# nihaomiao/CVPR23_LFDM

Measured on AMD Instinct MI355X. Metric: 40-frame 128x128 videos/sec (DDIM-100), higher is better.
Workload: dtype f32; 1 GPU; MUG 128x128, 40-frame DDIM-100 sample, batch=1 per GPU (BASELINE.json configs[1]); global_batch=1, frames=40, latent=32, image=128, sampler=DDIM-100 eta=1, cond_scale=1, parallelism=replicas x1 (videos sharded, no collective)

## Files before the change

cvpr23_lfdm_amd/csrc/lfdm_device.h:

```cpp
#pragma once
#include <stddef.h>
#include <stdint.h>
#include <type_traits>

#if defined(LFDM_EMU_BUILD)
#include "hip_emu.h"
typedef emu_f32x16 f32x16;
typedef emu_f32x4 f32x4;
#define LFDM_LAUNCH(kern, grid, block, smem, stream, ...) \
  emu::launch(grid, block, smem, [=]() { kern(__VA_ARGS__); })
static inline f32x16 mfma_32x32x2(float a, float b, f32x16 c) { return emu_mfma_32x32x2(a, b, c); }
static inline f32x4 mfma_16x16x4(float a, float b, f32x4 c) { return emu_mfma_16x16x4(a, b, c); }
static inline f32x4 mfma_4x4x1(float a, float b, f32x4 c) { return emu_mfma_4x4x1(a, b, c); }
struct lfdm_bf16x8 { uint16_t h[8]; };
static inline uint16_t lfdm_f32_to_bf16(float f) {
  uint32_t u;
  memcpy(&u, &f, 4);
  if ((u & 0x7fffffffu) > 0x7f800000u) return (uint16_t)((u >> 16) | 0x40u);
  u += 0x7fffu + ((u >> 16) & 1u);
  return (uint16_t)(u >> 16);
}
static inline float lfdm_bf16_to_f32(uint16_t h) {
  const uint32_t u = (uint32_t)h << 16;
  float f;
// ... 99 lines not shown
}
__device__ __forceinline__ float4 lfdm_buf_load_f4(lfdm_buf b, uint32_t off) {
  const lfdm_i32x4 v = __builtin_amdgcn_raw_buffer_load_b128(b, (int)off, 0, 0);
  float4 f;
  f.x = __int_as_float(v.x);
  f.y = __int_as_float(v.y);
  f.z = __int_as_float(v.z);
  f.w = __int_as_float(v.w);
  return f;
}
typedef int lfdm_i32x2 __attribute__((ext_vector_type(2)));
__device__ __forceinline__ float2 lfdm_buf_load_f2(lfdm_buf b, uint32_t off) {
  const lfdm_i32x2 v = __builtin_amdgcn_raw_buffer_load_b64(b, (int)off, 0, 0);
  return make_float2(__int_as_float(v.x), __int_as_float(v.y));
}
#endif
#define LFDM_BUF_OOB 0xFFFFFFF0u

#if defined(LFDM_EMU_BUILD)
static inline void lfdm_buf_store_f4_sc1(lfdm_buf b, uint32_t off, float4 v) {
  if ((uint64_t)off + 16u <= (uint64_t)b.bytes) memcpy(const_cast<char*>(b.base) + off, &v, 16);
}
static inline float4 lfdm_buf_load_f4_sc1(lfdm_buf b, uint32_t off) { return lfdm_buf_load_f4(b, off); }
#else
__device__ __forceinline__ void lfdm_buf_store_f4_sc1(lfdm_buf b, uint32_t off, float4 v) {
  lfdm_i32x4 d;
  d.x = __float_as_int(v.x); d.y = __float_as_int(v.y); d.z = __float_as_int(v.z); d.w = __float_as_int(v.w);
  __builtin_amdgcn_raw_buffer_store_b128(d, b, (int)off, 0, 16);
}
__device__ __forceinline__ float4 lfdm_buf_load_f4_sc1(lfdm_buf b, uint32_t off) {
  const lfdm_i32x4 v = __builtin_amdgcn_raw_buffer_load_b128(b, (int)off, 0, 16);
  float4 f;
  f.x = __int_as_float(v.x); f.y = __int_as_float(v.y); f.z = __int_as_float(v.z); f.w = __int_as_float(v.w);
  return f;
}
#endif

#if defined(LFDM_EMU_BUILD)
template <int OFF = 0> static inline void lfdm_gload_f4(f32x4& dst, const float* p) { memcpy(&dst, (const char*)p + OFF, 16); }
template <int N> static inline void lfdm_vmwait() {}
template <int N> static inline void lfdm_vmwait(f32x4&) {}
template <int N> static inline void lfdm_vmwait(f32x4&, f32x4&) {}
template <int N> static inline void lfdm_vmwait(f32x4&, f32x4&, f32x4&, f32x4&) {}
static inline void lfdm_tie(f32x4&) {}
static inline int lfdm_uniform(int v) { return v; }
#else
template <int OFF = 0>
__device__ __forceinline__ void lfdm_gload_f4(f32x4& dst, const float* p) {
  asm volatile("global_load_dwordx4 %0, %1, off offset:%2" : "=v"(dst) : "v"(p), "n"(OFF) : "memory");
}
template <int N> __device__ __forceinline__ void lfdm_vmwait() { asm volatile("s_waitcnt vmcnt(%0)" ::"n"(N) : "memory"); }
template <int N> __device__ __forceinline__ void lfdm_vmwait(f32x4& a) { asm volatile("s_waitcnt vmcnt(%1)" : "+v"(a) : "n"(N) : "memory"); }
template <int N> __device__ __forceinline__ void lfdm_vmwait(f32x4& a, f32x4& b) {
  asm volatile("s_waitcnt vmcnt(%2)" : "+v"(a), "+v"(b) : "n"(N) : "memory");
}
template <int N> __device__ __forceinline__ void lfdm_vmwait(f32x4& a, f32x4& b, f32x4& c, f32x4& d) {
  asm volatile("s_waitcnt vmcnt(%4)" : "+v"(a), "+v"(b), "+v"(c), "+v"(d) : "n"(N) : "memory");
// ... 87 lines not shown
```

cvpr23_lfdm_amd/csrc/linattn_fused.hip:

```cpp
#include <stdlib.h>

#include "lfdm_device.h"
#include "../../include/lfdm_hip.h"

namespace {

constexpr int HEADS = 8;
constexpr int DH = 32;
constexpr int OUT_LD = HEADS * DH;
constexpr int C = 64;
constexpr int CH = C / 2;
constexpr int SPLIT_TOK = 32;
constexpr int PART = DH * DH + 2 * DH;
constexpr float LA_SCALE = 0.17677669529663687f;

__device__ __forceinline__ void load_xraw(const float* __restrict__ xrow, int kh, float4 (&raw)[CH / 4]) {
#pragma unroll
  for (int q = 0; q < CH / 4; ++q) raw[q] = *reinterpret_cast<const float4*>(xrow + CH * kh + 4 * q);
}
__device__ __forceinline__ void xhat_stats(const float4 (&raw)[CH / 4], float eps, float& mean, float& rstd) {
  float s1 = 0.f, s2 = 0.f;
#pragma unroll
  for (int q = 0; q < CH / 4; ++q) {
    const float4 v = raw[q];
    s1 += (v.x + v.y) + (v.z + v.w);
    s2 += (v.x * v.x + v.y * v.y) + (v.z * v.z + v.w * v.w);
  }
  s1 += __shfl_xor(s1, 32);
  s2 += __shfl_xor(s2, 32);
  mean = s1 * (1.0f / (float)C);
  float var = s2 * (1.0f / (float)C) - mean * mean;
  if (var < 0.f) var = 0.f;
  rstd = 1.0f / sqrtf(var + eps);
}
__device__ __forceinline__ void xhat_apply(const float4 (&raw)[CH / 4], bool ok, float mean, float rstd, float (&xf)[CH]) {
#pragma unroll
// ... 2 lines not shown
    xf[4 * q] = ok ? (v.x - mean) * rstd : 0.f;
    xf[4 * q + 1] = ok ? (v.y - mean) * rstd : 0.f;
    xf[4 * q + 2] = ok ? (v.z - mean) * rstd : 0.f;
    xf[4 * q + 3] = ok ? (v.w - mean) * rstd : 0.f;
  }
}
__device__ __forceinline__ void load_xhat(const float* __restrict__ xrow, bool ok, int kh, float eps, float (&xf)[CH]) {
  float4 raw[CH / 4];
  float mean, rstd;
  load_xraw(xrow, kh, raw);
  xhat_stats(raw, eps, mean, rstd);
  xhat_apply(raw, ok, mean, rstd, xf);
}

__device__ __forceinline__ void load_wfrag(const float* __restrict__ wp, int which, int head, int lane, float (&wf)[CH]) {
  const float* src = wp + ((int64_t)(which * HEADS + head) * (CH / 4) * 64 + lane) * 4;
#pragma unroll
  for (int q = 0; q < CH / 4; ++q) {
    const float4 v = *reinterpret_cast<const float4*>(src + 256 * q);
    wf[4 * q] = v.x; wf[4 * q + 1] = v.y; wf[4 * q + 2] = v.z; wf[4 * q + 3] = v.w;
  }
}

__global__ __launch_bounds__(64, 3) void linattn_fused_ctx_kernel(const float* __restrict__ x, int ldx,
                                                                  const float* __restrict__ wqkv, int hw, float eps,
                                                                  float* __restrict__ part, int split_tok) {
  const int lane = threadIdx.x & 63, l31 = lane & 31, kh = lane >> 5;
  const int f = blockIdx.x >> 3, h = blockIdx.x & 7;
  const int split = blockIdx.y, nsplit = gridDim.y;
  const int n0 = split * split_tok;
  const int n1 = (n0 + split_tok < hw) ? n0 + split_tok : hw;

  float wk[CH], wv[CH];
  load_wfrag(wqkv, 1, h, lane, wk);
  load_wfrag(wqkv, 2, h, lane, wv);

  float m_run = -3.0e38f, s_run = 0.f;
  f32x16 ctx;
#pragma unroll
  for (int r = 0; r < 16; ++r) ctx[r] = 0.f;
  for (int t0 = n0; t0 < n1; t0 += 32) {
    const int n = t0 + l31;
    float xf[CH];
    load_xhat(x + ((int64_t)f * hw + (n < n1 ? n : n1 - 1)) * ldx, n < n1, kh, eps, xf);
    f32x16 ka, va;
#pragma unroll
    for (int r = 0; r < 16; ++r) ka[r] = va[r] = 0.f;
#pragma unroll
    for (int s = 0; s < CH; ++s) {
      ka = mfma_32x32x2(xf[s], wk[s], ka);
      va = mfma_32x32x2(xf[s], wv[s], va);
// ... 3 lines not shown
    for (int r = 0; r < 16; ++r) {
      const int tok = t0 + (r & 3) + 8 * (r >> 2) + 4 * kh;
      if (tok < n1) m = fmaxf(m, ka[r]);
    }
    m = fmaxf(m, __shfl_xor(m, 32));
    const float m_new = fmaxf(m_run, m);
    const float alpha = expf(m_run - m_new);
    float ssum = 0.f;
    float e[16];
#pragma unroll
    for (int r = 0; r < 16; ++r) {
      const int tok = t0 + (r & 3) + 8 * (r >> 2) + 4 * kh;
      e[r] = tok < n1 ? expf(ka[r] - m_new) : 0.f;
      ssum += e[r];
    }
    ssum += __shfl_xor(ssum, 32);
    s_run = s_run * alpha + ssum;
    m_run = m_new;
#pragma unroll
    for (int r = 0; r < 16; ++r) ctx[r] *= __shfl(alpha, (r & 3) + 8 * (r >> 2) + 4 * kh);
#pragma unroll
    for (int r = 0; r < 16; ++r) ctx = mfma_32x32x2(e[r], va[r], ctx);
  }
  float* dst = part + ((int64_t)blockIdx.x * nsplit + split) * PART;
#pragma unroll
  for (int r = 0; r < 16; ++r) dst[((r & 3) + 8 * (r >> 2) + 4 * kh) * DH + l31] = ctx[r];
  if (kh == 0) {
    dst[DH * DH + l31] = m_run;
    dst[DH * DH + DH + l31] = s_run;
  }
}

__global__ __launch_bounds__(256) void linattn_fused_merge_kernel(const float* __restrict__ part, int nsplit,
                                                                  float* __restrict__ ctx_out) {
  constexpr int MAXS = 64;
  __shared__ float s_w[MAXS][DH];
  const int tid = threadIdx.x;
  const float* base = part + (int64_t)blockIdx.x * nsplit * PART;
  if (nsplit <= 8) {
    constexpr int PS = 8;
    float cv[4][PS], pm[PS], psum[PS];
#pragma unroll
    for (int p = 0; p < PS; ++p) {
      const int pc = p < nsplit ? p : nsplit - 1;
#pragma unroll
      for (int e = 0; e < 4; ++e) cv[e][p] = base[(int64_t)pc * PART + tid + 256 * e];
      pm[p] = base[(int64_t)pc * PART + DH * DH + (tid & (DH - 1))];
      psum[p] = base[(int64_t)pc * PART + DH * DH + DH + (tid & (DH - 1))];
    }
    if (tid < DH) {
      float mm = -3.0e38f;
#pragma unroll
      for (int p = 0; p < PS; ++p)
        if (p < nsplit) mm = fmaxf(mm, pm[p]);
      float den = 0.f, w[PS];
#pragma unroll
      for (int p = 0; p < PS; ++p) {
        w[p] = p < nsplit ? expf(pm[p] - mm) : 0.f;
        den += w[p] * psum[p];
      }
      const float inv = 1.0f / den;
#pragma unroll
      for (int p = 0; p < PS; ++p)
        if (p < nsplit) s_w[p][tid] = w[p] * inv;
    }
    __syncthreads();
#pragma unroll
    for (int e = 0; e < 4; ++e) {
      const int i = tid + 256 * e, d = i >> 5;
      float acc = 0.f;
#pragma unroll
      for (int p = 0; p < PS; ++p)
        if (p < nsplit) acc += s_w[p][d] * cv[e][p];
      ctx_out[(int64_t)blockIdx.x * DH * DH + i] = acc;
    }
    return;
  }
  if (tid < DH) {
    float mm = -3.0e38f;
#pragma unroll 4
    for (int p = 0; p < nsplit; ++p) mm = fmaxf(mm, base[(int64_t)p * PART + DH * DH + tid]);
    float den = 0.f;
#pragma unroll 4
    for (int p = 0; p < nsplit; ++p) {
      const float w = expf(base[(int64_t)p * PART + DH * DH + tid] - mm);
      s_w[p][tid] = w;
      den += w * base[(int64_t)p * PART + DH * DH + DH + tid];
    }
    const float inv = 1.0f / den;
    for (int p = 0; p < nsplit; ++p) s_w[p][tid] *= inv;
  }
  __syncthreads();
  for (int i = tid; i < DH * DH; i += 256) {
    const int d = i >> 5;
    float acc = 0.f;
#pragma unroll 4
    for (int p = 0; p < nsplit; ++p) acc += s_w[p][d] * base[(int64_t)p * PART + i];
    ctx_out[(int64_t)blockIdx.x * DH * DH + i] = acc;
  }
}

__global__ __launch_bounds__(64, 2) void linattn_fused_out_kernel(const float* __restrict__ x, int ldx,
                                                                  const float* __restrict__ wqkv,
                                                                  const float* __restrict__ ctx, int hw, float eps,
                                                                  float* __restrict__ out) {
  const int lane = threadIdx.x & 63, l31 = lane & 31, kh = lane >> 5;
  const int f = blockIdx.y;
  const int n = blockIdx.x * 32 + l31;
  float xf[CH];
  load_xhat(x + ((int64_t)f * hw + (n < hw ? n : 0)) * ldx, n < hw, kh, eps, xf);
  const int hpb = HEADS / gridDim.z;
#pragma unroll 1
  for (int h = blockIdx.z * hpb; h < (blockIdx.z + 1) * hpb; ++h) {
    float wq[CH];
    load_wfrag(wqkv, 0, h, lane, wq);
    f32x16 q;
#pragma unroll
    for (int r = 0; r < 16; ++r) q[r] = 0.f;
#pragma unroll
    for (int s = 0; s < CH; ++s) q = mfma_32x32x2(wq[s], xf[s], q);
    float m = q[0];
#pragma unroll
    for (int r = 1; r < 16; ++r) m = fmaxf(m, q[r]);
    m = fmaxf(m, __shfl_xor(m, 32));
    float sum = 0.f;
#pragma unroll
    for (int r = 0; r < 16; ++r) {
      q[r] = expf(q[r] - m);
      sum += q[r];
    }
    sum += __shfl_xor(sum, 32);
    const float inv = LA_SCALE / sum;
    const float* cb = ctx + ((int64_t)f * HEADS + h) * DH * DH + l31;
    f32x16 o;
#pragma unroll
    for (int r = 0; r < 16; ++r) o[r] = 0.f;
#pragma unroll
    for (int r = 0; r < 16; ++r) o = mfma_32x32x2(q[r] * inv, cb[((r & 3) + 8 * (r >> 2) + 4 * kh) * DH], o);
#pragma unroll
    for (int r = 0; r < 16; ++r) {
      const int tok = blockIdx.x * 32 + (r & 3) + 8 * (r >> 2) + 4 * kh;
      if (tok < hw) out[((int64_t)f * hw + tok) * OUT_LD + h * DH + l31] = o[r];
    }
  }
}


constexpr int LDY = C + 4;
__global__ __launch_bounds__(256, 2) void linattn_fused_out2_kernel(const float* __restrict__ x, int ldx, const float* __restrict__ wqkv,
                                                                    const float* __restrict__ wout, const float* __restrict__ bias_out,
                                                                    const float* __restrict__ ctx, int hw, float eps, float* __restrict__ out,
                                                                    int ldo) {
  __shared__ __attribute__((aligned(16))) float s_y[4 * 32 * LDY];
  const int tid = threadIdx.x;
  const int wave = lfdm_uniform(tid >> 6);
  const int lane = tid & 63, l31 = lane & 31, kh = lane >> 5;
  const int f = blockIdx.y;
  const int n0 = blockIdx.x * 32;
  const int n = n0 + l31;
  float xf[CH];
  load_xhat(x + ((int64_t)f * hw + (n < hw ? n : 0)) * ldx, n < hw, kh, eps, xf);
  f32x16 yT[2];
#pragma unroll
  for (int cb = 0; cb < 2; ++cb)
#pragma unroll
    for (int r = 0; r < 16; ++r) yT[cb][r] = 0.f;
#pragma unroll 1
  for (int h = 2 * wave; h < 2 * wave + 2; ++h) {
    float wq[CH];
    load_wfrag(wqkv, 0, h, lane, wq);
    f32x16 q;
#pragma unroll
    for (int r = 0; r < 16; ++r) q[r] = 0.f;
#pragma unroll
    for (int s = 0; s < CH; ++s) q = mfma_32x32x2(wq[s], xf[s], q);
    float m = q[0];
#pragma unroll
    for (int r = 1; r < 16; ++r) m = fmaxf(m, q[r]);
    m = fmaxf(m, __shfl_xor(m, 32));
    float sum = 0.f;
#pragma unroll
    for (int r = 0; r < 16; ++r) {
      q[r] = expf(q[r] - m);
      sum += q[r];
    }
    sum += __shfl_xor(sum, 32);
    const float inv = LA_SCALE / sum;
    const float* cb_ = ctx + ((int64_t)f * HEADS + h) * DH * DH + l31;
    f32x16 oT;
#pragma unroll
    for (int r = 0; r < 16; ++r) oT[r] = 0.f;
#pragma unroll
    for (int r = 0; r < 16; ++r) oT = mfma_32x32x2(cb_[((r & 3) + 8 * (r >> 2) + 4 * kh) * DH], q[r] * inv, oT);
#pragma unroll
    for (int cb = 0; cb < 2; ++cb) {
      const float* wsrc = wout + ((int64_t)((h * 2 + cb) * 4) * 64 + lane) * 4;
      float4 wo[4];
#pragma unroll
      for (int qd = 0; qd < 4; ++qd) wo[qd] = *reinterpret_cast<const float4*>(wsrc + 256 * qd);
#pragma unroll
      for (int qd = 0; qd < 4; ++qd) {
        yT[cb] = mfma_32x32x2(wo[qd].x, oT[4 * qd + 0], yT[cb]);
        yT[cb] = mfma_32x32x2(wo[qd].y, oT[4 * qd + 1], yT[cb]);
        yT[cb] = mfma_32x32x2(wo[qd].z, oT[4 * qd + 2], yT[cb]);
        yT[cb] = mfma_32x32x2(wo[qd].w, oT[4 * qd + 3], yT[cb]);
      }
    }
  }
  float* ys = s_y + (wave * 32 + l31) * LDY;
#pragma unroll
  for (int cb = 0; cb < 2; ++cb)
#pragma unroll
    for (int g = 0; g < 4; ++g)
      *reinterpret_cast<float4*>(ys + 32 * cb + 8 * g + 4 * kh) = make_float4(yT[cb][4 * g], yT[cb][4 * g + 1], yT[cb][4 * g + 2], yT[cb][4 * g + 3]);
  __syncthreads();
  const int tok = tid >> 3, c8 = (tid & 7) * 8;
  if (n0 + tok < hw) {
    const int64_t row = (int64_t)f * hw + n0 + tok;
#pragma unroll
    for (int j = 0; j < 2; ++j) {
      const int c = c8 + 4 * j;
      float4 v = *reinterpret_cast<const float4*>(x + row * ldx + c);
      const float4 b4 = bias_out ? *reinterpret_cast<const float4*>(bias_out + c) : make_float4(0.f, 0.f, 0.f, 0.f);
      v.x += b4.x; v.y += b4.y; v.z += b4.z; v.w += b4.w;
#pragma unroll
      for (int w4 = 0; w4 < 4; ++w4) {
        const float4 u = *reinterpret_cast<const float4*>(s_y + (w4 * 32 + tok) * LDY + c);
        v.x += u.x; v.y += u.y; v.z += u.z; v.w += u.w;
      }
      *reinterpret_cast<float4*>(out + row * ldo + c) = v;
    }
  }
}

}

extern "C" size_t lfdm_linear_attention_fused_ws_bytes(int n_frames, int hw) {
  const int nsplit = (hw + SPLIT_TOK - 1) / SPLIT_TOK;
  return ((size_t)n_frames * HEADS * nsplit * PART + (size_t)n_frames * HEADS * DH * DH) * sizeof(float);
}

namespace {
void launch_ctx_and_merge(const float* x, int ldx, const float* wqkv, int n_frames, int hw, float ln_eps, void* ws, float** ctx_out,
                          hipStream_t stream) {
  const int tiles = (hw + 31) / 32;
  const int64_t pairs = (int64_t)n_frames * HEADS;
  int want = (int)((pairs <= 1536 ? 3072 : 4 * 3072 + pairs - 1) / pairs);
  if (const char* e = lfdm_knob("LFDM_LINATTN_SPLITS")) want = atoi(e);
  if (want < 1) want = 1;
  if (want > 64) want = 64;
  if (want > tiles) want = tiles;
  const int split_tok = ((tiles + want - 1) / want) * 32;
  const int nsplit = (hw + split_tok - 1) / split_tok;
  float* part = (float*)ws;
  float* ctx = part + (size_t)n_frames * HEADS * ((hw + SPLIT_TOK - 1) / SPLIT_TOK) * PART;
  LFDM_LAUNCH(linattn_fused_ctx_kernel, dim3(n_frames * HEADS, nsplit), dim3(64), 0, stream, x, ldx, wqkv, hw, ln_eps, part, split_tok);
  LFDM_LAUNCH(linattn_fused_merge_kernel, dim3(n_frames * HEADS), dim3(256), 0, stream, (const float*)part, nsplit, ctx);
  *ctx_out = ctx;
}
}

extern "C" int lfdm_linear_attention_fused_cl_f32(const float* x, int ldx, int channels, const float* wqkv, float* out,
                                                  int n_frames, int hw, float ln_eps, void* ws, size_t ws_bytes,
                                                  lfdm_stream_t stream_) {
  hipStream_t stream = (hipStream_t)stream_;
  if (!x || !wqkv || !out || n_frames <= 0 || hw <= 0 || hw > 64 * 64 || channels != C || ldx < C || ldx % 4 != 0 ||
      (((uintptr_t)x | (uintptr_t)wqkv) & 15) || (int64_t)n_frames * HEADS > 0x7fffffff) {
    lfdm_set_error("linear_attention_fused: needs C == 64 and 16-byte aligned rows");
    return LFDM_EINVAL;
  }
  if (!ws || ws_bytes < lfdm_linear_attention_fused_ws_bytes(n_frames, hw)) {
    lfdm_set_error("linear_attention_fused: workspace too small");
    return LFDM_EWORKSPACE;
  }
  float* ctx = nullptr;
  launch_ctx_and_merge(x, ldx, wqkv, n_frames, hw, ln_eps, ws, &ctx, stream);
  const int64_t otiles = (int64_t)((hw + 31) / 32) * n_frames;
  const int hgroups = otiles >= 4096 ? 1 : (otiles >= 2048 ? 2 : 4);
  LFDM_LAUNCH(linattn_fused_out_kernel, dim3((hw + 31) / 32, n_frames, hgroups), dim3(64), 0, stream, x, ldx, wqkv,
              (const float*)ctx, hw, ln_eps, out);
  return lfdm_check_launch("linear_attention_fused");
}

extern "C" int lfdm_linear_attention_fused_out_cl_f32(const float* x, int ldx, int channels, const float* wqkv, const float* wout,
                                                      const float* bias_out, float* out, int ldo, int n_frames, int hw, float ln_eps,
                                                      void* ws, size_t ws_bytes, lfdm_stream_t stream_) {
  hipStream_t stream = (hipStream_t)stream_;
  if (!x || !wqkv || !wout || !out || out == x || n_frames <= 0 || hw <= 0 || hw > 64 * 64 || channels != C || ldx < C || ldx % 4 != 0 || ldo < C ||
      ldo % 4 != 0 || (((uintptr_t)x | (uintptr_t)wqkv | (uintptr_t)wout | (uintptr_t)out | (uintptr_t)bias_out) & 15) ||
      (int64_t)n_frames * HEADS > 0x7fffffff || n_frames > 65535) {
    lfdm_set_error("linear_attention_fused_out: needs C == 64, 16-byte aligned rows, out != x, <= 65535 frames");
    return LFDM_EINVAL;
  }
  if (!ws || ws_bytes < lfdm_linear_attention_fused_ws_bytes(n_frames, hw)) {
    lfdm_set_error("linear_attention_fused_out: workspace too small");
    return LFDM_EWORKSPACE;
  }
  float* ctx = nullptr;
  launch_ctx_and_merge(x, ldx, wqkv, n_frames, hw, ln_eps, ws, &ctx, stream);
  LFDM_LAUNCH(linattn_fused_out2_kernel, dim3((hw + 31) / 32, n_frames), dim3(256), 0, stream, x, ldx, wqkv, wout, bias_out, (const float*)ctx, hw,
              ln_eps, out, ldo);
  return lfdm_check_launch("linear_attention_fused_out");
}
```

cvpr23_lfdm_amd/ops.py:

```python
import ctypes as C

import torch

from . import _native
from ._native import ConvParams, WarpParams

ACT_NONE, ACT_RELU, ACT_SIGMOID, ACT_SILU, ACT_GELU = 0, 1, 2, 3, 4


def _lib():
    return _native.library()


def _stream(lib):
    if lib.kind == "hip":
        return C.c_void_p(torch.cuda.current_stream().cuda_stream)
    return None


def _p(t):
    return None if t is None else C.c_void_p(t.data_ptr())


def _chk(lib, *tensors):
# ... 504 lines not shown
def temporal_attention_fused_out_cl(x, wqkv, wout, batch, frames, hw, *, bias=None, rot_cos=None, rot_sin=None, eps=1e-5, out=None):
    lib = _lib()
    _chk(lib, x, wqkv, wout, bias, rot_cos, rot_sin, out)
    c = x.shape[1]
    assert c == 64 and wqkv.shape == (3, 8, 2, 4, 64, 4) and wqkv.is_contiguous() and wout.shape == (4, 16, 64, 4) and wout.is_contiguous()
    if out is None:
        out = torch.empty(x.shape[0], c, dtype=torch.float32, device=x.device)
    assert out.data_ptr() != x.data_ptr()
    lib.check(lib.lfdm_temporal_attention_fused_out_cl_f32(_p(x), x.stride(0), c, _p(wqkv), _p(wout), _p(out), out.stride(0), batch, frames, hw,
                                                           _p(bias), _p(rot_cos), _p(rot_sin), eps, _stream(lib)),
              "lfdm_temporal_attention_fused_out_cl_f32")
    return out


def pack_linattn_weights(wqkv_folded):
    assert wqkv_folded.shape == (768, 64)
    return wqkv_folded.float().reshape(3, 8, 32, 2, 8, 4).permute(0, 1, 4, 3, 2, 5).contiguous().view(3, 8, 8, 64, 4)


def linear_attention_fused_ws_floats(n_frames, hw):
    return (int(_lib().lfdm_linear_attention_fused_ws_bytes(n_frames, hw)) + 3) // 4


def linear_attention_fused_cl(x, wqkv, n_frames, hw, *, eps=1e-5, out=None, ws=None):
    lib = _lib()
    _chk(lib, x, wqkv, out, ws)
    assert x.shape[1] == 64 and wqkv.shape == (3, 8, 8, 64, 4) and wqkv.is_contiguous()
    if out is None:
        out = torch.empty(x.shape[0], 256, dtype=torch.float32, device=x.device)
    need = lib.lfdm_linear_attention_fused_ws_bytes(n_frames, hw)
    if ws is not None:
        ws = ws.reshape(-1)
    if ws is None or ws.numel() * 4 < need:
        ws = torch.empty((need + 3) // 4, dtype=torch.float32, device=x.device)
    lib.check(lib.lfdm_linear_attention_fused_cl_f32(_p(x), x.stride(0), x.shape[1], _p(wqkv), _p(out), n_frames, hw, eps,
                                                     _p(ws), ws.numel() * 4, _stream(lib)),
              "lfdm_linear_attention_fused_cl_f32")
    return out


def pack_linattn_out_weight(wout):
    w = wout.float().reshape(64, 256)
    return w.reshape(2, 32, 8, 4, 2, 4).permute(2, 0, 3, 4, 1, 5).contiguous().view(8, 2, 4, 64, 4)


def linear_attention_fused_out_cl(x, wqkv, wout, bias_out, n_frames, hw, *, eps=1e-5, out=None, ws=None):
    lib = _lib()
    _chk(lib, x, wqkv, wout, bias_out, out, ws)
    assert x.shape[1] == 64 and wqkv.shape == (3, 8, 8, 64, 4) and wqkv.is_contiguous() and wout.shape == (8, 2, 4, 64, 4) and wout.is_contiguous()
    if out is None:
        out = torch.empty(x.shape[0], 64, dtype=torch.float32, device=x.device)
    assert out.data_ptr() != x.data_ptr()
    need = lib.lfdm_linear_attention_fused_ws_bytes(n_frames, hw)
    if ws is not None:
        ws = ws.reshape(-1)
    if ws is None or ws.numel() * 4 < need:
        ws = torch.empty((need + 3) // 4, dtype=torch.float32, device=x.device)
    lib.check(lib.lfdm_linear_attention_fused_out_cl_f32(_p(x), x.stride(0), x.shape[1], _p(wqkv), _p(wout), _p(bias_out), _p(out), out.stride(0),
                                                         n_frames, hw, eps, _p(ws), ws.numel() * 4, _stream(lib)),
              "lfdm_linear_attention_fused_out_cl_f32")
    return out


def linear_attention_lowres_cl(x, wqkv, wsum, n_frames, hw, *, eps=1e-5, out=None):
    lib = _lib()
    _chk(lib, x, wqkv, wsum, out)
    assert wqkv.shape == (768, x.shape[1]) and wqkv.is_contiguous() and wsum.numel() >= 768
    if out is None:
        out = torch.empty(x.shape[0], 256, dtype=torch.float32, device=x.device)
    lib.check(lib.lfdm_linear_attention_lowres_cl_f32(_p(x), x.stride(0), x.shape[1], _p(wqkv), _p(wsum), _p(out), n_frames, hw, eps,
                                                      _stream(lib)), "lfdm_linear_attention_lowres_cl_f32")
    return out


def linear_attention_lowres_ok(hw, channels):
    return channels % 64 == 0 and (hw <= 64 or 192 < hw <= 256)


def attention_lowres_cl(x, wqkv, wsum, batch, frames, hw, mode, *, bias=None, rot_cos=None, rot_sin=None, eps=1e-5, out=None):
    lib = _lib()
# ... 364 lines not shown
```

cvpr23_lfdm_amd/unet.py:

```python
import os

import torch
from torch import nn

from . import ops
from .params import ParamTree, build_tree, unet_spec, weights_epoch

BERT_MODEL_DIM = 768
MAX_FRAMES = 64


def check_num_frames(num_frames):
    if not 1 <= int(num_frames) <= MAX_FRAMES:
        raise ValueError("num_frames = %d: the temporal-attention kernels are built for 1 ... %d frames" % (int(num_frames), MAX_FRAMES))


_LOWRES_ATTN = os.environ.get("LFDM_LOWRES_ATTN", "1") != "0"
_LOWRES_MAX_HW = 64
_WINO_FUSE_REDUCE = os.environ.get("LFDM_WINO_FUSE_REDUCE", "1") != "0"
_TATTN_OUT = os.environ.get("LFDM_TATTN_OUT", "1") != "0"
_LINATTN_OUT = os.environ.get("LFDM_LINATTN_OUT", "1") != "0"
_RES_GN_MAX_ROWS = 65536
_RES_GN = os.environ.get("LFDM_RES_GN", "1") != "0"
_HEADS_GN = os.environ.get("LFDM_HEADS_GN", "1") != "0"
# ... 387 lines not shown
            att = self._buf("at.o", x.shape[0], 256)
            ops.temporal_attention_fused_cl(x, pk[prefix + "qkv.wf"], batch, frames, s * s, bias=bias, rot_cos=cos,
                                            rot_sin=sin, out=att)
        elif _LOWRES_ATTN and c % 64 == 0 and frames <= 64 and s * s <= _LOWRES_MAX_HW:
            att = self._buf("at.o", x.shape[0], 256)
            ops.attention_lowres_cl(x, pk[prefix + "qkv.wf"], pk[prefix + "qkv.wsum"], batch, frames, s * s, 0, bias=bias,
                                    rot_cos=cos, rot_sin=sin, out=att)
        else:
            qkv, att = self._attn_common(pk, prefix, x, batch * frames, s, c)
            ops.attention_cl(qkv, batch, frames, s * s, 0, bias=bias, rot_cos=cos, rot_sin=sin, out=att)
        out = self._buf(outname, x.shape[0], c)
        return self._conv(att, pk[prefix + "out.w"], c, 1, batch * frames, s, residual=x, out=out)

    def _spatial_attn(self, pk, prefix, x, batch, frames, s, c, outname):
        if _LOWRES_ATTN and c % 64 == 0 and s * s <= 64:
            att = self._buf("at.o", x.shape[0], 256)
            ops.attention_lowres_cl(x, pk[prefix + "qkv.wf"], pk[prefix + "qkv.wsum"], batch, frames, s * s, 1, out=att)
        else:
            qkv, att = self._attn_common(pk, prefix, x, batch * frames, s, c)
            ops.attention_cl(qkv, batch, frames, s * s, 1, out=att)
        out = self._buf(outname, x.shape[0], c)
        return self._conv(att, pk[prefix + "out.w"], c, 1, batch * frames, s, residual=x, out=out)

    def _linear_attn(self, pk, prefix, x, batch, frames, s, c, outname):
        n_img = batch * frames
        if c == 64 and _LINATTN_OUT:
            ws = self._buf("la.wsf", 1, ops.linear_attention_fused_ws_floats(n_img, s * s))
            return ops.linear_attention_fused_out_cl(x, pk[prefix + "qkv.wp"], pk[prefix + "out.wp"], pk[prefix + "out.b"], n_img, s * s,
                                                     out=self._buf(outname, x.shape[0], c), ws=ws)
        if c == 64:
            att = self._buf("at.o", x.shape[0], 256)
            ws = self._buf("la.wsf", 1, ops.linear_attention_fused_ws_floats(n_img, s * s))
            ops.linear_attention_fused_cl(x, pk[prefix + "qkv.wp"], n_img, s * s, out=att, ws=ws)
        elif _LOWRES_ATTN and ops.linear_attention_lowres_ok(s * s, c) and s * s <= _LOWRES_MAX_HW:
            att = self._buf("at.o", x.shape[0], 256)
            ops.linear_attention_lowres_cl(x, pk[prefix + "qkv.wf"], pk[prefix + "qkv.wsum"], n_img, s * s, out=att)
        else:
            qkv, att = self._attn_common(pk, prefix, x, n_img, s, c)
            ws = self._buf("la.ws", n_img, 8 * 32 * 32)
            ops.linear_attention_cl(qkv, n_img, s * s, out=att, ws=ws)
        out = self._buf(outname, x.shape[0], c)
        return self._conv(att, pk[prefix + "out.w"], c, 1, n_img, s, bias=pk[prefix + "out.b"], residual=x, out=out)

    def fea_term(self, pk, fea_cl, batch, s):
        return self._conv(fea_cl, pk["init.fea_w"], self.dim, 7, batch, s, bias=pk["init.b"],
                          out=self._buf("fea_term", batch * s * s, self.dim))

    def stem(self, pk, x_dyn, add_term, batch, frames, s):
        r = self._buf("r", batch * frames * s * s, self.dim)
        return ops.conv_planar_in_cl(x_dyn, batch, pk["n_dyn"], x_dyn.shape[1], frames, s, s, pk["init.dyn_w"],
                                     7, 7, self.dim, bias=None if add_term is not None else pk["init.b"],
                                     add_term=add_term, out=r)

    def run_trunk(self, pk, r, ss, batch, frames, s, out, focus=None):
        n_img = batch * frames
# ... 126 lines not shown
```

Baseline: 4.004 videos/s.

## Fuse linear-attention split merge into ctx kernel via tickets; pair out2 tiles

The separate merge kernel is removed. Each split block of the ctx kernel writes its partial context and takes an atomic ticket, and the last block for a frame/head merges all partials directly from registers using buffer loads. The out2 kernel can now process two token tiles per block, reusing the Wq, ctx and Wout fragments it loads with explicit vmcnt pipelining. Block indices are remapped for locality, and ticket counters live in a zeroed workspace prefix. This saves a launch and the merge's extra pass over global memory, at the cost of atomics, fences and serialized tail work in the last block.

```diff
diff --git a/cvpr23_lfdm_amd/csrc/lfdm_device.h b/cvpr23_lfdm_amd/csrc/lfdm_device.h
--- a/cvpr23_lfdm_amd/csrc/lfdm_device.h
+++ b/cvpr23_lfdm_amd/csrc/lfdm_device.h
@@ -145,6 +145,11 @@
   if ((uint64_t)off + 16u <= (uint64_t)b.bytes) memcpy(const_cast<char*>(b.base) + off, &v, 16);
 }
 static inline float4 lfdm_buf_load_f4_sc1(lfdm_buf b, uint32_t off) { return lfdm_buf_load_f4(b, off); }
+static inline float lfdm_buf_load_f1_sc1(lfdm_buf b, uint32_t off) {
+  float v = 0.f;
+  if ((uint64_t)off + 4u <= (uint64_t)b.bytes) memcpy(&v, b.base + off, 4);
+  return v;
+}
 #else
 __device__ __forceinline__ void lfdm_buf_store_f4_sc1(lfdm_buf b, uint32_t off, float4 v) {
   lfdm_i32x4 d;
@@ -156,6 +161,9 @@
   float4 f;
   f.x = __int_as_float(v.x); f.y = __int_as_float(v.y); f.z = __int_as_float(v.z); f.w = __int_as_float(v.w);
   return f;
+}
+__device__ __forceinline__ float lfdm_buf_load_f1_sc1(lfdm_buf b, uint32_t off) {
+  return __uint_as_float((unsigned)__builtin_amdgcn_raw_buffer_load_b32(b, (int)off, 0, 16));
 }
 #endif
 
diff --git a/cvpr23_lfdm_amd/csrc/linattn_fused.hip b/cvpr23_lfdm_amd/csrc/linattn_fused.hip
--- a/cvpr23_lfdm_amd/csrc/linattn_fused.hip
+++ b/cvpr23_lfdm_amd/csrc/linattn_fused.hip
@@ -12,6 +12,7 @@
 constexpr int CH = C / 2;
 constexpr int SPLIT_TOK = 32;
 constexpr int PART = DH * DH + 2 * DH;
+constexpr int CNT_ALIGN = 32;
 constexpr float LA_SCALE = 0.17677669529663687f;
 
 __device__ __forceinline__ void load_xraw(const float* __restrict__ xrow, int kh, float4 (&raw)[CH / 4]) {
@@ -60,11 +61,46 @@
   }
 }
 
+__device__ __forceinline__ int ctx_row(int r, int kh) { return (r & 3) + 8 * (r >> 2) + 4 * kh; }
+
+constexpr int MERGE_CHUNK = 4;
+__device__ __forceinline__ void ctx_merge_chunk(lfdm_buf pb, int p0, int nsplit, int lane, int l31, int kh, float mm, float inv, f32x16& acc) {
+  constexpr int PS = MERGE_CHUNK;
+  float4 cv[PS][4];
+  float pm[PS];
+#pragma unroll
+  for (int u = 0; u < PS; ++u) {
+    const int pc = p0 + u < nsplit ? p0 + u : nsplit - 1;
+#pragma unroll
+    for (int g = 0; g < 4; ++g) cv[u][g] = lfdm_buf_load_f4_sc1(pb, (uint32_t)((pc * PART + (g * 64 + lane) * 4) * 4));
+    pm[u] = lfdm_buf_load_f1_sc1(pb, (uint32_t)((pc * PART + DH * DH + l31) * 4));
+  }
+#pragma unroll
+  for (int u = 0; u < PS; ++u)
+    if (p0 + u < nsplit) {
+      const float w = expf(pm[u] - mm) * inv;
+#pragma unroll
+      for (int g = 0; g < 4; ++g) {
+        acc[4 * g + 0] += __shfl(w, ctx_row(4 * g + 0, kh)) * cv[u][g].x;
+        acc[4 * g + 1] += __shfl(w, ctx_row(4 * g + 1, kh)) * cv[u][g].y;
+        acc[4 * g + 2] += __shfl(w, ctx_row(4 * g + 2, kh)) * cv[u][g].z;
+        acc[4 * g + 3] += __shfl(w, ctx_row(4 * g + 3, kh)) * cv[u][g].w;
+      }
+    }
+}
+
 __global__ __launch_bounds__(64, 3) void linattn_fused_ctx_kernel(const float* __restrict__ x, int ldx,
                                                                   const float* __restrict__ wqkv, int hw, float eps,
-                                                                  float* __restrict__ part, int split_tok) {
+                                                                  float* __restrict__ part, int split_tok,
+                                                                  unsigned* __restrict__ tickets, float* __restrict__ ctx_out) {
   const int lane = threadIdx.x & 63, l31 = lane & 31, kh = lane >> 5;
-  const int f = blockIdx.x >> 3, h = blockIdx.x & 7;
+  int f = blockIdx.x >> 3, h = blockIdx.x & 7;
+  if ((int)blockIdx.x < (int)(gridDim.x & ~63u)) {
+    const int q = blockIdx.x >> 3;
+    f = (q & ~7) | (blockIdx.x & 7);
+    h = q & 7;
+  }
+  const int fh = f * HEADS + h;
   const int split = blockIdx.y, nsplit = gridDim.y;
   const int n0 = split * split_tok;
   const int n1 = (n0 + split_tok < hw) ? n0 + split_tok : hw;
@@ -114,81 +150,63 @@
 #pragma unroll
     for (int r = 0; r < 16; ++r) ctx = mfma_32x32x2(e[r], va[r], ctx);
   }
-  float* dst = part + ((int64_t)blockIdx.x * nsplit + split) * PART;
-#pragma unroll
-  for (int r = 0; r < 16; ++r) dst[((r & 3) + 8 * (r >> 2) + 4 * kh) * DH + l31] = ctx[r];
-  if (kh == 0) {
-    dst[DH * DH + l31] = m_run;
-    dst[DH * DH + DH + l31] = s_run;
-  }
-}
-
-__global__ __launch_bounds__(256) void linattn_fused_merge_kernel(const float* __restrict__ part, int nsplit,
-                                                                  float* __restrict__ ctx_out) {
-  constexpr int MAXS = 64;
-  __shared__ float s_w[MAXS][DH];
-  const int tid = threadIdx.x;
-  const float* base = part + (int64_t)blockIdx.x * nsplit * PART;
-  if (nsplit <= 8) {
-    constexpr int PS = 8;
-    float cv[4][PS], pm[PS], psum[PS];
+  const lfdm_buf pb = lfdm_make_buf(part + (int64_t)fh * nsplit * PART, (uint32_t)(nsplit * PART * 4));
+#pragma unroll
+  for (int g = 0; g < 4; ++g)
+    lfdm_buf_store_f4_sc1(pb, (uint32_t)((split * PART + (g * 64 + lane) * 4) * 4), make_float4(ctx[4 * g], ctx[4 * g + 1], ctx[4 * g + 2], ctx[4 * g + 3]));
+  {
+    const int src = 4 * (lane & 7);
+    const float4 mq = make_float4(__shfl(m_run, src), __shfl(m_run, src + 1), __shfl(m_run, src + 2), __shfl(m_run, src + 3));
+    const float4 sq = make_float4(__shfl(s_run, src), __shfl(s_run, src + 1), __shfl(s_run, src + 2), __shfl(s_run, src + 3));
+    if (lane < 16) lfdm_buf_store_f4_sc1(pb, (uint32_t)((split * PART + DH * DH + 4 * lane) * 4), lane < 8 ? mq : sq);
+  }
+  LFDM_DRAIN_STORES();
+  unsigned t = (unsigned)(nsplit - 1);
+  if (nsplit > 1 && lane == 0) {
+    t = lfdm_ticket_take(tickets + fh);
+    if (t == (unsigned)(nsplit - 1)) lfdm_ticket_reset(tickets + fh);
+  }
+  if (__shfl((int)t, 0) != nsplit - 1) return;
+  LFDM_FENCE_ACQUIRE_AGENT();
+  constexpr int PS = 8;
+  float mm = -3.0e38f, den = 0.f;
+  if (nsplit <= PS) {
+    float pm[PS], psum[PS];
 #pragma unroll
     for (int p = 0; p < PS; ++p) {
       const int pc = p < nsplit ? p : nsplit - 1;
-#pragma unroll
-      for (int e = 0; e < 4; ++e) cv[e][p] = base[(int64_t)pc * PART + tid + 256 * e];
-      pm[p] = base[(int64_t)pc * PART + DH * DH + (tid & (DH - 1))];
-      psum[p] = base[(int64_t)pc * PART + DH * DH + DH + (tid & (DH - 1))];
-    }
-    if (tid < DH) {
-      float mm = -3.0e38f;
-#pragma unroll
-      for (int p = 0; p < PS; ++p)
-        if (p < nsplit) mm = fmaxf(mm, pm[p]);
-      float den = 0.f, w[PS];
-#pragma unroll
-      for (int p = 0; p < PS; ++p) {
-        w[p] = p < nsplit ? expf(pm[p] - mm) : 0.f;
-        den += w[p] * psum[p];
-      }
-      const float inv = 1.0f / den;
-#pragma unroll
-      for (int p = 0; p < PS; ++p)
-        if (p < nsplit) s_w[p][tid] = w[p] * inv;
-    }
-    __syncthreads();
-#pragma unroll
-    for (int e = 0; e < 4; ++e) {
-      const int i = tid + 256 * e, d = i >> 5;
-      float acc = 0.f;
-#pragma unroll
-      for (int p = 0; p < PS; ++p)
-        if (p < nsplit) acc += s_w[p][d] * cv[e][p];
-      ctx_out[(int64_t)blockIdx.x * DH * DH + i] = acc;
-    }
-    return;
-  }
-  if (tid < DH) {
-    float mm = -3.0e38f;
+      pm[p] = lfdm_buf_load_f1_sc1(pb, (uint32_t)((pc * PART + DH * DH + l31) * 4));
+      psum[p] = lfdm_buf_load_f1_sc1(pb, (uint32_t)((pc * PART + DH * DH + DH + l31) * 4));
+    }
+#pragma unroll
+    for (int p = 0; p < PS; ++p)
+      if (p < nsplit) mm = fmaxf(mm, pm[p]);
+#pragma unroll
+    for (int p = 0; p < PS; ++p) den += (p < nsplit ? expf(pm[p] - mm) : 0.f) * psum[p];
+  } else {
 #pragma unroll 4
-    for (int p = 0; p < nsplit; ++p) mm = fmaxf(mm, base[(int64_t)p * PART + DH * DH + tid]);
-    float den = 0.f;
+    for (int p = 0; p < nsplit; ++p) mm = fmaxf(mm, lfdm_buf_load_f1_sc1(pb, (uint32_t)((p * PART + DH * DH + l31) * 4)));
 #pragma unroll 4
-    for (int p = 0; p < nsplit; ++p) {
-      const float w = expf(base[(int64_t)p * PART + DH * DH + tid] - mm);
-      s_w[p][tid] = w;
-      den += w * base[(int64_t)p * PART + DH * DH + DH + tid];
-    }
-    const float inv = 1.0f / den;
-    for (int p = 0; p < nsplit; ++p) s_w[p][tid] *= inv;
-  }
-  __syncthreads();
-  for (int i = tid; i < DH * DH; i += 256) {
-    const int d = i >> 5;
-    float acc = 0.f;
-#pragma unroll 4
-    for (int p = 0; p < nsplit; ++p) acc += s_w[p][d] * base[(int64_t)p * PART + i];
-    ctx_out[(int64_t)blockIdx.x * DH * DH + i] = acc;
+    for (int p = 0; p < nsplit; ++p)
+      den += expf(lfdm_buf_load_f1_sc1(pb, (uint32_t)((p * PART + DH * DH + l31) * 4)) - mm) *
+             lfdm_buf_load_f1_sc1(pb, (uint32_t)((p * PART + DH * DH + DH + l31) * 4));
+  }
+  const float inv = 1.0f / den;
+  f32x16 acc;
+#pragma unroll
+  for (int r = 0; r < 16; ++r) acc[r] = 0.f;
+  for (int p0 = 0; p0 < nsplit; p0 += MERGE_CHUNK) ctx_merge_chunk(pb, p0, nsplit, lane, l31, kh, mm, inv, acc);
+  float* dst = ctx_out + (int64_t)fh * DH * DH + lane * 4;
+#pragma unroll
+  for (int g = 0; g < 4; ++g) *reinterpret_cast<float4*>(dst + 256 * g) = make_float4(acc[4 * g], acc[4 * g + 1], acc[4 * g + 2], acc[4 * g + 3]);
+}
+
+__device__ __forceinline__ void load_ctxfrag(const float* __restrict__ ctx, int64_t fh, int lane, float (&cf)[16]) {
+  const float* src = ctx + fh * DH * DH + lane * 4;
+#pragma unroll
+  for (int g = 0; g < 4; ++g) {
+    const float4 v = *reinterpret_cast<const float4*>(src + 256 * g);
+    cf[4 * g] = v.x; cf[4 * g + 1] = v.y; cf[4 * g + 2] = v.z; cf[4 * g + 3] = v.w;
   }
 }
 
@@ -223,12 +241,13 @@
     }
     sum += __shfl_xor(sum, 32);
     const float inv = LA_SCALE / sum;
-    const float* cb = ctx + ((int64_t)f * HEADS + h) * DH * DH + l31;
+    float cf[16];
+    load_ctxfrag(ctx, (int64_t)f * HEADS + h, lane, cf);
     f32x16 o;
 #pragma unroll
     for (int r = 0; r < 16; ++r) o[r] = 0.f;
 #pragma unroll
-    for (int r = 0; r < 16; ++r) o = mfma_32x32x2(q[r] * inv, cb[((r & 3) + 8 * (r >> 2) + 4 * kh) * DH], o);
+    for (int r = 0; r < 16; ++r) o = mfma_32x32x2(q[r] * inv, cf[r], o);
 #pragma unroll
     for (int r = 0; r < 16; ++r) {
       const int tok = blockIdx.x * 32 + (r & 3) + 8 * (r >> 2) + 4 * kh;
@@ -239,102 +258,164 @@
 
 
 constexpr int LDY = C + 4;
+constexpr int OUT2_SLOTS = 512;
+template <int NT>
+__device__ __forceinline__ void out2_tiles(const float* __restrict__ x, int ldx, const float* __restrict__ wqkv, const float* __restrict__ wout,
+                                           const float* __restrict__ bias_out, const float* __restrict__ ctx, int hw, float eps,
+                                           float* __restrict__ out, int ldo, int f, int tile0, float* s_y) {
+  const int tid = threadIdx.x;
+  const int wave = lfdm_uniform(tid >> 6);
+  const int lane = tid & 63, l31 = lane & 31, kh = lane >> 5;
+  f32x4 wq[2][8], cf[2][4], wo[2][2][4];
+  const auto req_wq = [&](int hh) {
+    const float* src = wqkv + ((int64_t)(2 * wave + hh) * (CH / 4) * 64 + lane) * 4;
+    lfdm_gload_f4<0>(wq[hh][0], src); lfdm_gload_f4<1024>(wq[hh][1], src); lfdm_gload_f4<2048>(wq[hh][2], src); lfdm_gload_f4<3072>(wq[hh][3], src);
+    lfdm_gload_f4<0>(wq[hh][4], src + 1024); lfdm_gload_f4<1024>(wq[hh][5], src + 1024); lfdm_gload_f4<2048>(wq[hh][6], src + 1024);
+    lfdm_gload_f4<3072>(wq[hh][7], src + 1024);
+  };
+  const auto req_cf = [&](int hh) {
+    const float* src = ctx + ((int64_t)f * HEADS + 2 * wave + hh) * DH * DH + lane * 4;
+    lfdm_gload_f4<0>(cf[hh][0], src); lfdm_gload_f4<1024>(cf[hh][1], src); lfdm_gload_f4<2048>(cf[hh][2], src); lfdm_gload_f4<3072>(cf[hh][3], src);
+  };
+  const auto req_wo = [&](int hh, int cb) {
+    const float* src = wout + ((int64_t)(((2 * wave + hh) * 2 + cb) * 4) * 64 + lane) * 4;
+    lfdm_gload_f4<0>(wo[hh][cb][0], src); lfdm_gload_f4<1024>(wo[hh][cb][1], src); lfdm_gload_f4<2048>(wo[hh][cb][2], src);
+    lfdm_gload_f4<3072>(wo[hh][cb][3], src);
+  };
+  req_wq(0);
+  float xf[NT][CH];
+#pragma unroll
+  for (int t = 0; t < NT; ++t) {
+    const int n = (tile0 + t) * 32 + l31;
+    load_xhat(x + ((int64_t)f * hw + (n < hw ? n : 0)) * ldx, n < hw, kh, eps, xf[t]);
+  }
+  f32x16 yT[NT][2];
+#pragma unroll
+  for (int t = 0; t < NT; ++t)
+#pragma unroll
+    for (int cb = 0; cb < 2; ++cb)
+#pragma unroll
+      for (int r = 0; r < 16; ++r) yT[t][cb][r] = 0.f;
+  lfdm_static_for<0, 2>([&](auto hh_) {
+    constexpr int hh = decltype(hh_)::value;
+    constexpr bool more = hh == 0;
+    lfdm_vmwait<0>(wq[hh][0], wq[hh][1], wq[hh][2], wq[hh][3]);
+    lfdm_vmwait<0>(wq[hh][4], wq[hh][5], wq[hh][6], wq[hh][7]);
+    req_cf(hh);
+    req_wo(hh, 0);
+    f32x16 q[NT];
+#pragma unroll
+    for (int t = 0; t < NT; ++t)
+#pragma unroll
+      for (int r = 0; r < 16; ++r) q[t][r] = 0.f;
+#pragma unroll
+    for (int s = 0; s < CH; ++s)
+#pragma unroll
+      for (int t = 0; t < NT; ++t) q[t] = mfma_32x32x2(wq[hh][s >> 2][s & 3], xf[t][s], q[t]);
+    float inv[NT];
+#pragma unroll
+    for (int t = 0; t < NT; ++t) {
+      float m = q[t][0];
+#pragma unroll
+      for (int r = 1; r < 16; ++r) m = fmaxf(m, q[t][r]);
+      m = fmaxf(m, __shfl_xor(m, 32));
+      float sum = 0.f;
+#pragma unroll
+      for (int r = 0; r < 16; ++r) {
+        q[t][r] = expf(q[t][r] - m);
+        sum += q[t][r];
+      }
+      sum += __shfl_xor(sum, 32);
+      inv[t] = LA_SCALE / sum;
+    }
+    lfdm_vmwait<4>(cf[hh][0], cf[hh][1], cf[hh][2], cf[hh][3]);
+    f32x16 oT[NT];
+#pragma unroll
+    for (int t = 0; t < NT; ++t)
+#pragma unroll
+      for (int r = 0; r < 16; ++r) oT[t][r] = 0.f;
+#pragma unroll
+    for (int r = 0; r < 16; ++r)
+#pragma unroll
+      for (int t = 0; t < NT; ++t) oT[t] = mfma_32x32x2(cf[hh][r >> 2][r & 3], q[t][r] * inv[t], oT[t]);
+    req_wo(hh, 1);
+    if constexpr (more) req_wq(hh + 1);
+#pragma unroll
+    for (int cb = 0; cb < 2; ++cb) {
+      if (cb == 0) {
+        lfdm_vmwait<more ? 12 : 4>(wo[hh][0][0], wo[hh][0][1], wo[hh][0][2], wo[hh][0][3]);
+      } else {
+        lfdm_vmwait<more ? 8 : 0>(wo[hh][1][0], wo[hh][1][1], wo[hh][1][2], wo[hh][1][3]);
+      }
+#pragma unroll
+      for (int qd = 0; qd < 4; ++qd) {
+#pragma unroll
+        for (int i = 0; i < 4; ++i)
+#pragma unroll
+          for (int t = 0; t < NT; ++t) yT[t][cb] = mfma_32x32x2(wo[hh][cb][qd][i], oT[t][4 * qd + i], yT[t][cb]);
+      }
+    }
+  });
+#pragma unroll
+  for (int t = 0; t < NT; ++t) {
+    if (t > 0) __syncthreads();
+    float* ys = s_y + (wave * 32 + l31) * LDY;
+#pragma unroll
+    for (int cb = 0; cb < 2; ++cb)
+#pragma unroll
+      for (int g = 0; g < 4; ++g)
+        *reinterpret_cast<float4*>(ys + 32 * cb + 8 * g + 4 * kh) =
+            make_float4(yT[t][cb][4 * g], yT[t][cb][4 * g + 1], yT[t][cb][4 * g + 2], yT[t][cb][4 * g + 3]);
+    __syncthreads();
+    const int n0 = (tile0 + t) * 32;
+    const int tok = tid >> 3, c8 = (tid & 7) * 8;
+    if (n0 + tok < hw) {
+      const int64_t row = (int64_t)f * hw + n0 + tok;
+#pragma unroll
+      for (int j = 0; j < 2; ++j) {
+        const int c = c8 + 4 * j;
+        float4 v = *reinterpret_cast<const float4*>(x + row * ldx + c);
+        const float4 b4 = bias_out ? *reinterpret_cast<const float4*>(bias_out + c) : make_float4(0.f, 0.f, 0.f, 0.f);
+        v.x += b4.x; v.y += b4.y; v.z += b4.z; v.w += b4.w;
+#pragma unroll
+        for (int w4 = 0; w4 < 4; ++w4) {
+          const float4 u = *reinterpret_cast<const float4*>(s_y + (w4 * 32 + tok) * LDY + c);
+          v.x += u.x; v.y += u.y; v.z += u.z; v.w += u.w;
+        }
+        *reinterpret_cast<float4*>(out + row * ldo + c) = v;
+      }
+    }
+  }
+}
+
 __global__ __launch_bounds__(256, 2) void linattn_fused_out2_kernel(const float* __restrict__ x, int ldx, const float* __restrict__ wqkv,
                                                                     const float* __restrict__ wout, const float* __restrict__ bias_out,
                                                                     const float* __restrict__ ctx, int hw, float eps, float* __restrict__ out,
-                                                                    int ldo) {
+                                                                    int ldo, int npair, int ppf) {
   __shared__ __attribute__((aligned(16))) float s_y[4 * 32 * LDY];
-  const int tid = threadIdx.x;
-  const int wave = lfdm_uniform(tid >> 6);
-  const int lane = tid & 63, l31 = lane & 31, kh = lane >> 5;
-  const int f = blockIdx.y;
-  const int n0 = blockIdx.x * 32;
-  const int n = n0 + l31;
-  float xf[CH];
-  load_xhat(x + ((int64_t)f * hw + (n < hw ? n : 0)) * ldx, n < hw, kh, eps, xf);
-  f32x16 yT[2];
-#pragma unroll
-  for (int cb = 0; cb < 2; ++cb)
-#pragma unroll
-    for (int r = 0; r < 16; ++r) yT[cb][r] = 0.f;
-#pragma unroll 1
-  for (int h = 2 * wave; h < 2 * wave + 2; ++h) {
-    float wq[CH];
-    load_wfrag(wqkv, 0, h, lane, wq);
-    f32x16 q;
-#pragma unroll
-    for (int r = 0; r < 16; ++r) q[r] = 0.f;
-#pragma unroll
-    for (int s = 0; s < CH; ++s) q = mfma_32x32x2(wq[s], xf[s], q);
-    float m = q[0];
-#pragma unroll
-    for (int r = 1; r < 16; ++r) m = fmaxf(m, q[r]);
-    m = fmaxf(m, __shfl_xor(m, 32));
-    float sum = 0.f;
-#pragma unroll
-    for (int r = 0; r < 16; ++r) {
-      q[r] = expf(q[r] - m);
-      sum += q[r];
-    }
-    sum += __shfl_xor(sum, 32);
-    const float inv = LA_SCALE / sum;
-    const float* cb_ = ctx + ((int64_t)f * HEADS + h) * DH * DH + l31;
-    f32x16 oT;
-#pragma unroll
-    for (int r = 0; r < 16; ++r) oT[r] = 0.f;
-#pragma unroll
-    for (int r = 0; r < 16; ++r) oT = mfma_32x32x2(cb_[((r & 3) + 8 * (r >> 2) + 4 * kh) * DH], q[r] * inv, oT);
-#pragma unroll
-    for (int cb = 0; cb < 2; ++cb) {
-      const float* wsrc = wout + ((int64_t)((h * 2 + cb) * 4) * 64 + lane) * 4;
-      float4 wo[4];
-#pragma unroll
-      for (int qd = 0; qd < 4; ++qd) wo[qd] = *reinterpret_cast<const float4*>(wsrc + 256 * qd);
-#pragma unroll
-      for (int qd = 0; qd < 4; ++qd) {
-        yT[cb] = mfma_32x32x2(wo[qd].x, oT[4 * qd + 0], yT[cb]);
-        yT[cb] = mfma_32x32x2(wo[qd].y, oT[4 * qd + 1], yT[cb]);
-        yT[cb] = mfma_32x32x2(wo[qd].z, oT[4 * qd + 2], yT[cb]);
-        yT[cb] = mfma_32x32x2(wo[qd].w, oT[4 * qd + 3], yT[cb]);
-      }
-    }
-  }
-  float* ys = s_y + (wave * 32 + l31) * LDY;
-#pragma unroll
-  for (int cb = 0; cb < 2; ++cb)
-#pragma unroll
-    for (int g = 0; g < 4; ++g)
-      *reinterpret_cast<float4*>(ys + 32 * cb + 8 * g + 4 * kh) = make_float4(yT[cb][4 * g], yT[cb][4 * g + 1], yT[cb][4 * g + 2], yT[cb][4 * g + 3]);
-  __syncthreads();
-  const int tok = tid >> 3, c8 = (tid & 7) * 8;
-  if (n0 + tok < hw) {
-    const int64_t row = (int64_t)f * hw + n0 + tok;
-#pragma unroll
-    for (int j = 0; j < 2; ++j) {
-      const int c = c8 + 4 * j;
-      float4 v = *reinterpret_cast<const float4*>(x + row * ldx + c);
-      const float4 b4 = bias_out ? *reinterpret_cast<const float4*>(bias_out + c) : make_float4(0.f, 0.f, 0.f, 0.f);
-      v.x += b4.x; v.y += b4.y; v.z += b4.z; v.w += b4.w;
-#pragma unroll
-      for (int w4 = 0; w4 < 4; ++w4) {
-        const float4 u = *reinterpret_cast<const float4*>(s_y + (w4 * 32 + tok) * LDY + c);
-        v.x += u.x; v.y += u.y; v.z += u.z; v.w += u.w;
-      }
-      *reinterpret_cast<float4*>(out + row * ldo + c) = v;
-    }
-  }
-}
-
-}
+  const int id = blockIdx.x, tiles = (hw + 31) >> 5;
+  const bool pair = id < npair;
+  const int u = pair ? id : npair + ((id - npair) >> 1);
+  const int f = u / ppf;
+  const int tile0 = 2 * (u - f * ppf) + (pair ? 0 : ((id - npair) & 1));
+  if (tile0 >= tiles) return;
+  if (pair && tile0 + 1 < tiles)
+    out2_tiles<2>(x, ldx, wqkv, wout, bias_out, ctx, hw, eps, out, ldo, f, tile0, s_y);
+  else
+    out2_tiles<1>(x, ldx, wqkv, wout, bias_out, ctx, hw, eps, out, ldo, f, tile0, s_y);
+}
+
+}
+
+static size_t ws_ticket_words(int n_frames) { return ((size_t)n_frames * HEADS + CNT_ALIGN - 1) / CNT_ALIGN * CNT_ALIGN; }
 
 extern "C" size_t lfdm_linear_attention_fused_ws_bytes(int n_frames, int hw) {
   const int nsplit = (hw + SPLIT_TOK - 1) / SPLIT_TOK;
-  return ((size_t)n_frames * HEADS * nsplit * PART + (size_t)n_frames * HEADS * DH * DH) * sizeof(float);
+  return (ws_ticket_words(n_frames) + (size_t)n_frames * HEADS * nsplit * PART + (size_t)n_frames * HEADS * DH * DH) * sizeof(float);
 }
 
 namespace {
-void launch_ctx_and_merge(const float* x, int ldx, const float* wqkv, int n_frames, int hw, float ln_eps, void* ws, float** ctx_out,
-                          hipStream_t stream) {
+void launch_ctx(const float* x, int ldx, const float* wqkv, int n_frames, int hw, float ln_eps, void* ws, float** ctx_out, hipStream_t stream) {
   const int tiles = (hw + 31) / 32;
   const int64_t pairs = (int64_t)n_frames * HEADS;
   int want = (int)((pairs <= 1536 ? 3072 : 4 * 3072 + pairs - 1) / pairs);
@@ -344,11 +425,21 @@
   if (want > tiles) want = tiles;
   const int split_tok = ((tiles + want - 1) / want) * 32;
   const int nsplit = (hw + split_tok - 1) / split_tok;
-  float* part = (float*)ws;
+  unsigned* tickets = (unsigned*)ws;
+  float* part = (float*)ws + ws_ticket_words(n_frames);
   float* ctx = part + (size_t)n_frames * HEADS * ((hw + SPLIT_TOK - 1) / SPLIT_TOK) * PART;
-  LFDM_LAUNCH(linattn_fused_ctx_kernel, dim3(n_frames * HEADS, nsplit), dim3(64), 0, stream, x, ldx, wqkv, hw, ln_eps, part, split_tok);
-  LFDM_LAUNCH(linattn_fused_merge_kernel, dim3(n_frames * HEADS), dim3(256), 0, stream, (const float*)part, nsplit, ctx);
+  LFDM_LAUNCH(linattn_fused_ctx_kernel, dim3(n_frames * HEADS, nsplit), dim3(64), 0, stream, x, ldx, wqkv, hw, ln_eps, part, split_tok, tickets, ctx);
   *ctx_out = ctx;
+}
+
+void launch_out2(const float* x, int ldx, const float* wqkv, const float* wout, const float* bias_out, const float* ctx, int n_frames, int hw,
+                 float ln_eps, float* out, int ldo, hipStream_t stream) {
+  const int tiles = (hw + 31) / 32, ppf = (tiles + 1) / 2;
+  const int64_t units = (int64_t)n_frames * ppf;
+  int64_t npair = (int64_t)n_frames * tiles <= OUT2_SLOTS ? 0 : (units < OUT2_SLOTS ? units : OUT2_SLOTS);
+  if (const char* e = lfdm_knob("LFDM_LINATTN_OUT2_PAIRS")) npair = atol(e) < units ? atol(e) : units;
+  LFDM_LAUNCH(linattn_fused_out2_kernel, dim3((unsigned)(npair + 2 * (units - npair))), dim3(256), 0, stream, x, ldx, wqkv, wout, bias_out, ctx, hw,
+              ln_eps, out, ldo, (int)npair, ppf);
 }
 }
 
@@ -366,7 +457,7 @@
     return LFDM_EWORKSPACE;
   }
   float* ctx = nullptr;
-  launch_ctx_and_merge(x, ldx, wqkv, n_frames, hw, ln_eps, ws, &ctx, stream);
+  launch_ctx(x, ldx, wqkv, n_frames, hw, ln_eps, ws, &ctx, stream);
   const int64_t otiles = (int64_t)((hw + 31) / 32) * n_frames;
   const int hgroups = otiles >= 4096 ? 1 : (otiles >= 2048 ? 2 : 4);
   LFDM_LAUNCH(linattn_fused_out_kernel, dim3((hw + 31) / 32, n_frames, hgroups), dim3(64), 0, stream, x, ldx, wqkv,
@@ -389,8 +480,7 @@
     return LFDM_EWORKSPACE;
   }
   float* ctx = nullptr;
-  launch_ctx_and_merge(x, ldx, wqkv, n_frames, hw, ln_eps, ws, &ctx, stream);
-  LFDM_LAUNCH(linattn_fused_out2_kernel, dim3((hw + 31) / 32, n_frames), dim3(256), 0, stream, x, ldx, wqkv, wout, bias_out, (const float*)ctx, hw,
-              ln_eps, out, ldo);
+  launch_ctx(x, ldx, wqkv, n_frames, hw, ln_eps, ws, &ctx, stream);
+  launch_out2(x, ldx, wqkv, wout, bias_out, ctx, n_frames, hw, ln_eps, out, ldo, stream);
   return lfdm_check_launch("linear_attention_fused_out");
 }
diff --git a/cvpr23_lfdm_amd/ops.py b/cvpr23_lfdm_amd/ops.py
--- a/cvpr23_lfdm_amd/ops.py
+++ b/cvpr23_lfdm_amd/ops.py
@@ -550,6 +550,16 @@
     return (int(_lib().lfdm_linear_attention_fused_ws_bytes(n_frames, hw)) + 3) // 4
 
 
+def linear_attention_fused_ws_ticket_words(n_frames):
+    return (n_frames * 8 + 31) // 32 * 32
+
+
+def linear_attention_fused_ws(n_frames, hw, device):
+    ws = torch.empty(linear_attention_fused_ws_floats(n_frames, hw), dtype=torch.float32, device=device)
+    ws[:linear_attention_fused_ws_ticket_words(n_frames)].zero_()
+    return ws
+
+
 def linear_attention_fused_cl(x, wqkv, n_frames, hw, *, eps=1e-5, out=None, ws=None):
     lib = _lib()
     _chk(lib, x, wqkv, out, ws)
@@ -560,7 +570,7 @@
     if ws is not None:
         ws = ws.reshape(-1)
     if ws is None or ws.numel() * 4 < need:
-        ws = torch.empty((need + 3) // 4, dtype=torch.float32, device=x.device)
+        ws = linear_attention_fused_ws(n_frames, hw, x.device)
     lib.check(lib.lfdm_linear_attention_fused_cl_f32(_p(x), x.stride(0), x.shape[1], _p(wqkv), _p(out), n_frames, hw, eps,
                                                      _p(ws), ws.numel() * 4, _stream(lib)),
               "lfdm_linear_attention_fused_cl_f32")
@@ -583,7 +593,7 @@
     if ws is not None:
         ws = ws.reshape(-1)
     if ws is None or ws.numel() * 4 < need:
-        ws = torch.empty((need + 3) // 4, dtype=torch.float32, device=x.device)
+        ws = linear_attention_fused_ws(n_frames, hw, x.device)
     lib.check(lib.lfdm_linear_attention_fused_out_cl_f32(_p(x), x.stride(0), x.shape[1], _p(wqkv), _p(wout), _p(bias_out), _p(out), out.stride(0),
                                                          n_frames, hw, eps, _p(ws), ws.numel() * 4, _stream(lib)),
               "lfdm_linear_attention_fused_out_cl_f32")
diff --git a/cvpr23_lfdm_amd/unet.py b/cvpr23_lfdm_amd/unet.py
--- a/cvpr23_lfdm_amd/unet.py
+++ b/cvpr23_lfdm_amd/unet.py
@@ -433,15 +433,24 @@
         out = self._buf(outname, x.shape[0], c)
         return self._conv(att, pk[prefix + "out.w"], c, 1, batch * frames, s, residual=x, out=out)
 
+    def _linattn_ws(self, n_img, hw):
+        need = ops.linear_attention_fused_ws_floats(n_img, hw)
+        gen = self._buf_gen
+        ws = self._buf("la.wsf", 1, need)
+        if gen != self._buf_gen or getattr(self, "_la_ws_frames", None) != n_img:
+            self._bufs["la.wsf"][:ops.linear_attention_fused_ws_ticket_words(n_img)].zero_()
+            self._la_ws_frames = n_img
+        return ws
+
     def _linear_attn(self, pk, prefix, x, batch, frames, s, c, outname):
         n_img = batch * frames
         if c == 64 and _LINATTN_OUT:
-            ws = self._buf("la.wsf", 1, ops.linear_attention_fused_ws_floats(n_img, s * s))
+            ws = self._linattn_ws(n_img, s * s)
             return ops.linear_attention_fused_out_cl(x, pk[prefix + "qkv.wp"], pk[prefix + "out.wp"], pk[prefix + "out.b"], n_img, s * s,
                                                      out=self._buf(outname, x.shape[0], c), ws=ws)
         if c == 64:
             att = self._buf("at.o", x.shape[0], 256)
-            ws = self._buf("la.wsf", 1, ops.linear_attention_fused_ws_floats(n_img, s * s))
+            ws = self._linattn_ws(n_img, s * s)
             ops.linear_attention_fused_cl(x, pk[prefix + "qkv.wp"], n_img, s * s, out=att, ws=ws)
         elif _LOWRES_ATTN and ops.linear_attention_lowres_ok(s * s, c) and s * s <= _LOWRES_MAX_HW:
             att = self._buf("at.o", x.shape[0], 256)
```

New measurement: 4.027 videos/s, median of 6. Within noise of the previous version (+0.6%).
